# nfmoore/databricks-kubernetes-mlops-poc

Measured on NVIDIA H100. Metric: rows/sec at batch=65536x23f, higher is better.
Workload: dtype u16 ranks + f64acc

## Files before the change

databricks_kubernetes_mlops_poc_b200/csrc/b2f_api.cu:

```cuda
#include <cuda_runtime.h>
#include <dlfcn.h>
#include <limits.h>
#include <nccl.h>
#include <stdarg.h>
#include <stddef.h>
#include <stdio.h>
#include <stdlib.h>
#include <string.h>

#include <algorithm>
#include <cmath>
#include <string>
#include <thread>
#include <new>
#include <vector>

#include "../../include/b2f.h"
#include "feature_moments.cuh"
#include "forest_blob.h"
#include "forest_predict.cuh"
#include "forest_predict_tile.cuh"
#include "forest_predict_rank.cuh"
#include "forest_rank.h"
#include "tree_shap.cuh"
// ... 204 lines not shown
                const uint32_t t = N[(s * 32 + l) * 2], m = N[(s * 32 + l) * 2 + 1];
                const uint32_t feat = m >> B2F_META_FEAT_SHIFT, first = m & B2F_META_SLOT_MASK;
                const bool leaf = (first == s);
                if ((m & 0x03000000u) || feat > B2F_SENTINEL_WORD)
                    return set_err(B2F_EINVAL, "forest blob: group %u slot %u lane %u: bad meta word 0x%08x", g, s, l, m);
                if (leaf) {
                    if (!(m & B2F_META_CAT) || feat != B2F_SENTINEL_WORD || t >= gr.n_leaf_slots)
                        return set_err(B2F_EINVAL, "forest blob: group %u slot %u lane %u: malformed leaf", g, s, l);
                } else {
                    if (first <= s || first + 1 >= gr.n_slots) return set_err(B2F_EINVAL, "forest blob: group %u slot %u lane %u: child %u out of range", g, s, l, first);
                    if ((m & B2F_META_CAT) && feat >= h.n_cat && feat != B2F_SENTINEL_WORD)
                        return set_err(B2F_EINVAL, "forest blob: group %u slot %u lane %u: categorical test on numeric word", g, s, l);
                }
            }
    }
    if (expect_off != h.chunks_bytes) return set_err(B2F_EINVAL, "forest blob: chunks_bytes mismatch");
    *hdr_out = h;
    return B2F_OK;
}

extern "C" int b2f_blob_validate(const void *forest_blob, size_t nbytes) {
    b2f_blob_header h;
    return validate_blob(static_cast<const uint8_t *>(forest_blob), nbytes, &h);
}

extern "C" b2f_ranker *b2f_ranker_create(const void *forest_blob, size_t nbytes) {
    b2f_blob_header h;
    if (validate_blob(static_cast<const uint8_t *>(forest_blob), nbytes, &h) != B2F_OK) return nullptr;
    b2f_ranker *r = new (std::nothrow) b2f_ranker();
    if (!r) {
        set_err(B2F_ENOMEM, "out of host memory");
        return nullptr;
    }
    ranker_build(r, static_cast<const uint8_t *>(forest_blob), h);
    return r;
}
extern "C" void b2f_ranker_destroy(b2f_ranker *r) { delete r; }

static void fill_rank_info(const b2f_ranker *r, bool ok, b2f_rank_info *out) {
    memset(out, 0, sizeof(*out));
    out->ok = ok ? 1 : 0;
    out->row_bytes = r->row_bytes;
    out->cat_bytes = r->cat_bytes;
    out->n_cat = r->n_cat;
    out->n_num = r->n_num;
    out->depth = r->depth;
    out->n_trees = r->n_trees;
    out->layout_bytes = (int32_t)r->layout.size();
    for (int j = 0; j < 16; ++j) {
        out->cat_shift[j] = r->cat_shift[j];
        out->cat_bits[j] = r->cat_bits[j];
    }
    for (size_t k = 0; k < r->thr.size() && k < 24; ++k) out->n_thresholds[k] = (int32_t)r->thr[k].size();
    out->n_pairs = (int32_t)r->pairs.size();
    for (size_t i = 0; i < r->pairs.size() && i < 128; ++i) out->pairs[i] = r->pairs[i];
    snprintf(out->why, sizeof(out->why), "%s", r->why);
}
extern "C" int b2f_ranker_info(const b2f_ranker *r, b2f_rank_info *out) {
    if (!r || !out) return set_err(B2F_EINVAL, "null argument");
    fill_rank_info(r, r->ok, out);
    return B2F_OK;
}
extern "C" const float *b2f_ranker_thresholds(const b2f_ranker *r, int k, int32_t *count) {
    if (!r || k < 0 || k >= (int)r->thr.size()) {
        if (count) *count = 0;
        return nullptr;
    }
    if (count) *count = (int32_t)r->thr[k].size();
    return r->thr[k].data();
}
extern "C" const void *b2f_ranker_layout(const b2f_ranker *r, int64_t *nbytes) {
    if (!r || !r->ok) {
        if (nbytes) *nbytes = 0;
        return nullptr;
    }
    if (nbytes) *nbytes = (int64_t)r->layout.size();
    return r->layout.data();
}
extern "C" int b2f_ranker_rank_rows(const b2f_ranker *r, const void *rows, int64_t n, int row_format, void *ranked_out, int threads) {
    if (!r || n < 0 || (n > 0 && (!rows || !ranked_out))) return set_err(B2F_EINVAL, "bad argument");
    if (!r->ok) return set_err(B2F_EINVAL, "no rank layout for this forest (%s)", r->why);
    if (row_format != B2F_ROWS_WORDS24 && row_format != B2F_ROWS_PACKED64) return set_err(B2F_EINVAL, "rows must be B2F_ROWS_WORDS24 or B2F_ROWS_PACKED64");
    if (row_format == B2F_ROWS_PACKED64 && !(r->n_cat == 9 && r->n_num <= 14)) return set_err(B2F_EINVAL, "schema does not fit the packed 64-byte row");
    threads = (int)std::min<int64_t>(std::max(threads, 1), std::max<int64_t>(1, n / 4096));
    const uint8_t *in = static_cast<const uint8_t *>(rows);
    uint8_t *out = static_cast<uint8_t *>(ranked_out);
    if (threads == 1) {
        rank_rows_range(r, in, 0, n, row_format, out);
        return B2F_OK;
    }
    std::vector<std::thread> pool;
    for (int t = 1; t < threads; ++t) pool.emplace_back([=] { rank_rows_range(r, in, n * t / threads, n * (t + 1) / threads, row_format, out); });
    rank_rows_range(r, in, 0, n / threads, row_format, out);
    for (auto &th : pool) th.join();
    return B2F_OK;
}

template <typename OutT>
using RankKernel = void (*)(RParams, const uint8_t *, long long, OutT *, int32_t *, int);

template <int R, typename OutT>
static auto warp_kernel_r(bool smem, bool pk) {
    if (smem) return pk ? k_forest_predict<R, true, true, OutT> : k_forest_predict<R, true, false, OutT>;
    return pk ? k_forest_predict<R, false, true, OutT> : k_forest_predict<R, false, false, OutT>;
}
template <typename OutT>
static auto warp_kernel(int rows_per_warp, bool smem, bool pk) {
    if (rows_per_warp == 4) return warp_kernel_r<4, OutT>(smem, pk);
    return rows_per_warp == 2 ? warp_kernel_r<2, OutT>(smem, pk) : warp_kernel_r<1, OutT>(smem, pk);
}
template <typename OutT>
static auto tile_kernel(bool pk) {
    return pk ? k_forest_predict_tile<true, OutT> : k_forest_predict_tile<false, OutT>;
}
template <typename OutT>
static auto split_kernel(bool pk) {
    return pk ? k_forest_predict_split<2, true, OutT> : k_forest_predict_split<2, false, OutT>;
}
template <typename OutT, int D = 1>
static RankKernel<OutT> rank_kernel(const b2f_model *m) {
    if constexpr (D > 8) {
        return nullptr;
    } else {
        if (m->rp.depth != D) return rank_kernel<OutT, D + 1>(m);
        if (m->rank_stream) return k_forest_predict_rank<D, 4, true, OutT>;
        return m->rank_u == 8 ? k_forest_predict_rank<D, 8, false, OutT> : k_forest_predict_rank<D, 4, false, OutT>;
    }
}
template <typename K>
static cudaError_t set_smem_limit(K kernel, int bytes) {
    return kernel ? cudaFuncSetAttribute(kernel, cudaFuncAttributeMaxDynamicSharedMemorySize, bytes) : cudaErrorInvalidValue;
}

enum { KN_AUTO, KN_WARP, KN_TILE, KN_SPLIT };
struct EnvHooks {
    int kernel = KN_AUTO;
    bool walk_global = false;
    bool walk_smem = false;
    int64_t chunk_rows = B2F_CHUNK_ROWS;
    std::vector<int64_t> chunk_plan{768};
    int64_t split_max_rows = 2048;
    int rows_per_warp = 2;
    int64_t tile_min_rows = -1;
    int tile_warps = 0;
    bool rank_off = false;
    int rank_max_tiles = INT_MAX;
    int rank_stream = -1;
    int rank_u = 4;
    bool rank_wait_first = false;
    bool no_pdl = false;
};

static EnvHooks read_env_hooks(void) {
    EnvHooks h;
    if (const char *v = getenv("B2F_KERNEL"))
        h.kernel = !strcmp(v, "warp") ? KN_WARP : !strcmp(v, "tile") ? KN_TILE : !strcmp(v, "split") ? KN_SPLIT : KN_AUTO;
    if (const char *v = getenv("B2F_FORCE_WALK")) {
        h.walk_global = !strcmp(v, "global");
        h.walk_smem = !strcmp(v, "smem");
    }
    if (const char *v = getenv("B2F_CHUNK_ROWS"))
        if (atoll(v) >= 1024) h.chunk_rows = atoll(v);
    if (const char *v = getenv("B2F_CHUNK_PLAN")) {
        h.chunk_plan.clear();
        for (const char *q = v; *q;) {
            h.chunk_plan.push_back(atoll(q));
            while (*q && *q != ',') ++q;
            if (*q == ',') ++q;
        }
    }
    if (const char *v = getenv("B2F_SPLIT_MAX_ROWS")) h.split_max_rows = atoll(v);
    if (const char *v = getenv("B2F_ROWS_PER_WARP")) {
        const int r = atoi(v);
        if (r == 1 || r == 2 || r == 4) h.rows_per_warp = r;
    }
    if (const char *v = getenv("B2F_TILE_MIN_ROWS"))
        if (atoll(v) >= 0) h.tile_min_rows = atoll(v);
    if (const char *v = getenv("B2F_TILE_WARPS")) h.tile_warps = std::min(B2F_TILE_WARPS_MAX, std::max(1, atoi(v)));
    if (const char *v = getenv("B2F_RANK")) h.rank_off = !strcmp(v, "0");
    if (const char *v = getenv("B2F_RANK_MAX_TILES")) h.rank_max_tiles = std::max(1, atoi(v));
    if (const char *v = getenv("B2F_RANK_STREAM")) h.rank_stream = atoi(v) != 0;
    if (const char *v = getenv("B2F_RANK_U")) h.rank_u = atoi(v) == 8 ? 8 : 4;
    if (const char *v = getenv("B2F_RANK_WAIT_FIRST")) h.rank_wait_first = atoi(v) != 0;
    h.no_pdl = getenv("B2F_NO_PDL") != nullptr;
    return h;
}


struct TileTree {
    std::vector<uint32_t> nodes;
    std::vector<double> leaves;
    uint32_t depth = 0;
};

static bool extract_tree(const uint8_t *blob, const b2f_blob_header &h, const b2f_blob_group &gr, uint32_t lane, TileTree &out) {
    const uint32_t *N = reinterpret_cast<const uint32_t *>(blob + h.chunks_off + gr.chunk_off);
    const double *LV = reinterpret_cast<const double *>(blob + h.chunks_off + gr.chunk_off + (size_t)gr.n_slots * 256);
    std::vector<uint32_t> depth_of(gr.n_slots, 0);
    uint32_t reach = 0, max_leaf = 0, max_depth = 0;
    for (uint32_t s = 0; s <= reach; ++s) {
        const uint32_t t = N[(s * 32 + lane) * 2], m = N[(s * 32 + lane) * 2 + 1];
        const uint32_t feat = m >> B2F_META_FEAT_SHIFT, first = m & B2F_META_SLOT_MASK;
        const bool cat = (m & B2F_META_CAT) != 0;
        if (first >= B2F_TILE_MAX_TREE_NODES) return false;
        out.nodes.push_back(t);
        out.nodes.push_back((first << B2F_TILE_CHILD_SHIFT) | (cat ? B2F_TILE_META_CAT : 0u) | (feat << B2F_TILE_FEAT_SHIFT));
        if (first == s) {
            max_leaf = std::max(max_leaf, t);
            max_depth = std::max(max_depth, depth_of[s]);
        } else {
            reach = std::max(reach, first + 1);
            depth_of[first] = depth_of[first + 1] = depth_of[s] + 1;
        }
    }
    out.leaves.resize(max_leaf + 1);
    for (uint32_t i = 0; i <= max_leaf; ++i) out.leaves[i] = LV[i * 32 + lane];
    out.depth = max_depth;
    return true;
}

static bool build_tile_layout(const uint8_t *blob, const b2f_blob_header &h, uint32_t avail_smem, std::vector<uint8_t> &layout,
                              std::vector<TPiece> &pieces, uint32_t *slot_bytes, int *n_slots) {
    const b2f_blob_group *gt = reinterpret_cast<const b2f_blob_group *>(blob + h.groups_off);
    std::vector<TileTree> trees(h.n_trees);
    for (uint32_t t = 0; t < h.n_trees; ++t)
        if (!extract_tree(blob, h, gt[t / 32], t % 32, trees[t])) return false;
    struct UG {
        uint32_t first, count, bytes;
    };
    std::vector<UG> ugs;
    uint64_t total = 0;
    for (uint32_t t = 0; t < h.n_trees; t += B2F_TILE_U) {
        UG u{t, std::min<uint32_t>(B2F_TILE_U, h.n_trees - t), (uint32_t)sizeof(TUGroup)};
        for (uint32_t k = 0; k < B2F_TILE_U; ++k)
            u.bytes += k < u.count ? (uint32_t)(trees[t + k].nodes.size() * 4 + trees[t + k].leaves.size() * 8) : 16u;
        ugs.push_back(u);
        total += u.bytes;
    }
    uint32_t max_ug = 0;
    for (const UG &u : ugs) max_ug = std::max(max_ug, u.bytes);
    const bool fits = total + (uint64_t)(max_ug + 128) * B2F_TILE_MAX_SLOTS <= avail_smem;
    uint32_t target = fits ? (uint32_t)((total + B2F_TILE_MAX_SLOTS - 1) / B2F_TILE_MAX_SLOTS) + max_ug : 32u * 1024u;
    layout.clear();
    pieces.clear();
    size_t i = 0;
    uint32_t max_piece = 0;
    while (i < ugs.size()) {
        size_t j = i;
        uint32_t bytes = 0;
        while (j < ugs.size() && (j == i || bytes + ugs[j].bytes <= target)) bytes += ugs[j++].bytes;
        const uint32_t n_ug = (uint32_t)(j - i);
        const size_t start = layout.size();
        std::vector<uint8_t> buf((size_t)n_ug * sizeof(TUGroup));
        for (uint32_t g = 0; g < n_ug; ++g) {
            TUGroup d;
            memset(&d, 0, sizeof(d));
            for (uint32_t k = 0; k < B2F_TILE_U; ++k) {
                while (buf.size() % 8) buf.push_back(0);
                d.node_off[k] = (uint32_t)buf.size();
                if (k < ugs[i + g].count) {
                    const TileTree &tr = trees[ugs[i + g].first + k];
                    const uint8_t *np = reinterpret_cast<const uint8_t *>(tr.nodes.data());
                    buf.insert(buf.end(), np, np + tr.nodes.size() * 4);
                    d.leaf_off[k] = (uint32_t)buf.size();
                    const uint8_t *lp = reinterpret_cast<const uint8_t *>(tr.leaves.data());
                    buf.insert(buf.end(), lp, lp + tr.leaves.size() * 8);
                    d.depth = std::max(d.depth, tr.depth);
                } else {
                    const uint32_t stub[2] = {0u, (0u << B2F_TILE_CHILD_SHIFT) | B2F_TILE_META_CAT | (B2F_SENTINEL_WORD << B2F_TILE_FEAT_SHIFT)};
                    const uint8_t *sp = reinterpret_cast<const uint8_t *>(stub);
                    buf.insert(buf.end(), sp, sp + 8);
                    d.leaf_off[k] = (uint32_t)buf.size();
                    const double z = 0.0;
                    const uint8_t *zp = reinterpret_cast<const uint8_t *>(&z);
                    buf.insert(buf.end(), zp, zp + 8);
                }
            }
            memcpy(buf.data() + (size_t)g * sizeof(TUGroup), &d, sizeof(d));
        }
        while (buf.size() % 128) buf.push_back(0);
        layout.insert(layout.end(), buf.begin(), buf.end());
        pieces.push_back(TPiece{(uint32_t)start, (uint32_t)buf.size(), n_ug, 0u});
        max_piece = std::max<uint32_t>(max_piece, (uint32_t)buf.size());
        i = j;
    }
    *slot_bytes = max_piece;
    if ((size_t)max_piece * pieces.size() <= avail_smem && pieces.size() <= B2F_TILE_MAX_SLOTS) {
        *n_slots = (int)pieces.size();
    } else {
        int s = (int)std::min<uint64_t>(B2F_TILE_MAX_SLOTS, avail_smem / max_piece);
        if (s < 2) return false;
        *n_slots = s;
    }
    return true;
}

static int rank_init(b2f_model *m, const uint8_t *blob, const EnvHooks &env) {
    m->rank_ok = false;
    ranker_build(&m->rk, blob, m->hdr);
    if (!m->rk.ok) return B2F_OK;
    if (env.rank_off) return B2F_OK;
    const int64_t layout_bytes = (int64_t)m->rk.layout.size();
    const int64_t base = B2F_RANK_XS_BYTES  + (int64_t)B2F_RANK_PARTIALS * 32 * 8 + 256;
    int max_tiles = (int)std::min<int64_t>(B2F_RANK_MAX_TILES, ((int64_t)m->max_smem_optin - base - layout_bytes) / B2F_RANK_XS_BYTES);
    max_tiles = std::min(max_tiles, env.rank_max_tiles);
    m->rank_stream = env.rank_stream < 0 ? max_tiles < 8 : env.rank_stream != 0;
    int64_t forest_smem = layout_bytes;
    m->rank_u = env.rank_u;
    if (m->rank_stream) {
        m->rank_u = 4;
        const int64_t piece = 8 * (int64_t)m->rk.tree_stride;
        forest_smem = 2 * piece;
        max_tiles = (int)std::min<int64_t>(B2F_RANK_MAX_TILES, ((int64_t)m->max_smem_optin - base - forest_smem) / B2F_RANK_XS_BYTES);
        if (max_tiles < 4 || piece % 16) return B2F_OK;
    }
    CUDA_TRY(cudaMalloc(&m->d_rank_layout, (size_t)layout_bytes));
    CUDA_TRY(cudaMemcpy(m->d_rank_layout, m->rk.layout.data(), (size_t)layout_bytes, cudaMemcpyHostToDevice));
    RParams &rp = m->rp;
    memset(&rp, 0, sizeof(rp));
    rp.layout = static_cast<const uint8_t *>(m->d_rank_layout);
    rp.layout_bytes = (uint32_t)layout_bytes;
    rp.tree_stride = m->rk.tree_stride;
    rp.n_trees_padded = m->rk.n_trees_padded;
    rp.depth = m->rk.depth;
    rp.agg_mode = (int)m->hdr.agg_mode;
    rp.n_cat = m->rk.n_cat;
    rp.n_num = m->rk.n_num;
    rp.row_bytes = m->rk.row_bytes;
    rp.cat_bytes = m->rk.cat_bytes;
    rp.max_tiles = max_tiles;
    rp.groups_per_piece = 2;
    rp.piece_bytes = 8u * m->rk.tree_stride;
    rp.n_pieces = m->rk.n_trees_padded / 8;
    rp.init_raw = m->hdr.init_raw;
    rp.denom = m->hdr.denom;
    rp.threshold = m->hdr.threshold;
    rp.mul_two = 2u;
    rp.mul_64k = 65536u;
    rp.add_64k = 65535u;
    rp.n_pairs = (int)m->rk.pairs.size();
    rp.wait_first = env.rank_wait_first;
    m->rank_pdl = !env.no_pdl;
    for (int j = 0; j < 16; ++j) {
        rp.cat_shift[j] = (uint8_t)m->rk.cat_shift[j];
        rp.cat_bits[j] = (uint8_t)m->rk.cat_bits[j];
        rp.cat_start[j] = 0;
        rp.cat_mask[j] = 0ull;
    }
    for (int i = rp.n_pairs - 1; i >= 0; --i) {
        const uint32_t j = m->rk.pairs[i] >> 16, c = m->rk.pairs[i] & 0xFFFFu;
        rp.cat_start[j] = (uint8_t)i;
        rp.cat_mask[j] |= 1ull << c;
    }
    m->rank_smem_bytes = (int)(B2F_RANK_XS_BYTES + (int64_t)max_tiles * B2F_RANK_XS_BYTES + (int64_t)B2F_RANK_PARTIALS * 32 * 8 + forest_smem);
    CUDA_TRY(set_smem_limit(rank_kernel<float>(m), m->rank_smem_bytes));
    CUDA_TRY(set_smem_limit(rank_kernel<double>(m), m->rank_smem_bytes));
    m->rank_ok = true;
    return B2F_OK;
}

static int warp_init(b2f_model *m, const uint8_t *blob, const EnvHooks &env) {
    KParams &kp = m->kp;
    memset(&kp, 0, sizeof(kp));
    kp.chunks = static_cast<const uint8_t *>(m->d_blob) + m->hdr.chunks_off;
    kp.n_groups = (int)m->hdr.n_groups;
    kp.agg_mode = (int)m->hdr.agg_mode;
    kp.n_cat = (int)m->hdr.n_cat;
    kp.n_num = (int)m->hdr.n_num;
    kp.init_raw = m->hdr.init_raw;
    kp.denom = m->hdr.denom;
    kp.threshold = m->hdr.threshold;
    memcpy(kp.impute, m->hdr.impute, sizeof(kp.impute));
    const b2f_blob_group *gt = reinterpret_cast<const b2f_blob_group *>(blob + m->hdr.groups_off);
    for (uint32_t g = 0; g < m->hdr.n_groups; ++g) {
        kp.g[g].chunk_off = gt[g].chunk_off;
        kp.g[g].chunk_bytes = gt[g].chunk_bytes;
        kp.g[g].n_slots = gt[g].n_slots;
        kp.g[g].n_leaf_slots = gt[g].n_leaf_slots;
        kp.g[g].depth = gt[g].depth;
    }

    m->packed_ok = m->hdr.n_cat == 9 && m->hdr.n_num <= 14;
    for (uint32_t f = 0; f < m->hdr.n_cat; ++f)
        if (m->hdr.vocab[f] > 126) m->packed_ok = false;

    const int64_t need = (int64_t)m->hdr.chunks_bytes;
    const bool fits = need + 1024 <= (int64_t)m->max_smem_optin && !env.walk_global;
    if (env.walk_smem && !fits) return set_err(B2F_EINVAL, "B2F_FORCE_WALK=smem but forest needs %lld bytes", (long long)need);
    m->walk_mode = fits ? B2F_WALK_SMEM : B2F_WALK_GLOBAL;
    m->smem_bytes = fits ? (int)need : 0;
    if (fits)
        for (bool pk : {false, true})
            for (int r : {1, 2, 4}) {
                CUDA_TRY(set_smem_limit(warp_kernel<float>(r, true, pk), m->smem_bytes));
                CUDA_TRY(set_smem_limit(warp_kernel<double>(r, true, pk), m->smem_bytes));
            }
    m->chunk_rows = env.chunk_rows;
    m->chunk_plan = env.chunk_plan;
    m->split_max_rows = env.split_max_rows;
    if (env.kernel == KN_WARP || env.kernel == KN_TILE) m->split_max_rows = 0;
    if (env.kernel == KN_SPLIT) m->split_max_rows = INT64_MAX;
    m->rows_per_warp_max = env.rows_per_warp;
    return B2F_OK;
}

static int tile_init(b2f_model *m, const uint8_t *blob, const EnvHooks &env) {
    std::vector<uint8_t> layout;
    std::vector<TPiece> pieces;
    uint32_t slot_bytes = 0;
    int n_slots = 0;
    bool ok = false;
    int cwarps = B2F_TILE_WARPS_MIN;
    const int w_hi = env.tile_warps ? env.tile_warps : B2F_TILE_WARPS_MAX, w_lo = env.tile_warps ? env.tile_warps : B2F_TILE_WARPS_MIN;
    for (int w = w_hi; env.kernel != KN_WARP && w >= w_lo && !ok; w -= 4) {
        const uint32_t avail = (uint32_t)m->max_smem_optin - 1024u - 4096u - (uint32_t)w * B2F_TILE_XS_BYTES;
        const bool built = build_tile_layout(blob, m->hdr, avail, layout, pieces, &slot_bytes, &n_slots);
        const bool res = built && (int)pieces.size() <= n_slots;
        if (built && (res || w == w_lo)) {
            ok = true;
            cwarps = w;
        }
    }
    if (!ok) {
        if (env.kernel == KN_TILE) return set_err(B2F_EINVAL, "B2F_KERNEL=tile but the forest's trees do not fit the tile kernel's shared-memory ring");
        return B2F_OK;
    }
    CUDA_TRY(cudaMalloc(&m->d_tile_layout, layout.size()));
    CUDA_TRY(cudaMemcpy(m->d_tile_layout, layout.data(), layout.size(), cudaMemcpyHostToDevice));
    CUDA_TRY(cudaMalloc((void **)&m->d_tile_pieces, pieces.size() * sizeof(TPiece)));
    CUDA_TRY(cudaMemcpy(m->d_tile_pieces, pieces.data(), pieces.size() * sizeof(TPiece), cudaMemcpyHostToDevice));
    const KParams &kp = m->kp;
    TParams &tp = m->tp;
    memset(&tp, 0, sizeof(tp));
    tp.layout = static_cast<const uint8_t *>(m->d_tile_layout);
    tp.pieces = m->d_tile_pieces;
    tp.n_pieces = (int)pieces.size();
    tp.n_slots = n_slots;
    tp.slot_bytes = slot_bytes;
    tp.agg_mode = kp.agg_mode;
    tp.n_cat = kp.n_cat;
    tp.n_num = kp.n_num;
    tp.init_raw = kp.init_raw;
    tp.denom = kp.denom;
    tp.threshold = kp.threshold;
    memcpy(tp.impute, kp.impute, sizeof(tp.impute));
    m->tile_cwarps = cwarps;
    m->tile_smem_bytes = 4096 + cwarps * B2F_TILE_XS_BYTES + n_slots * (int)slot_bytes;
    m->tile_layout_bytes = (int64_t)layout.size();
    for (bool pk : {false, true}) {
        CUDA_TRY(set_smem_limit(tile_kernel<float>(pk), m->tile_smem_bytes));
        CUDA_TRY(set_smem_limit(tile_kernel<double>(pk), m->tile_smem_bytes));
    }
    m->tile_ok = true;
    m->tile_min_rows = (tp.n_pieces <= tp.n_slots) ? 65536 : 24576;
    if (env.tile_min_rows >= 0) m->tile_min_rows = env.tile_min_rows;
    if (env.kernel == KN_TILE) m->tile_min_rows = 1;
    return B2F_OK;
}

static int streams_init(b2f_model *m) {
    for (int s = 0; s < B2F_STREAMS; ++s) CUDA_TRY(cudaStreamCreateWithFlags(&m->slots[s].stream, cudaStreamNonBlocking));
    CUDA_TRY(cudaStreamCreateWithFlags(&m->compute, cudaStreamNonBlocking));
    CUDA_TRY(cudaFuncSetAttribute(k_feature_moments, cudaFuncAttributeMaxDynamicSharedMemorySize, B2F_MOM_SMEM));
    m->mom_blocks = m->sm_count * 3;
    CUDA_TRY(cudaMalloc(&m->d_mom_partials, (size_t)m->mom_blocks * B2F_MOM_VALUES * sizeof(double)));
    CUDA_TRY(cudaMalloc(&m->d_mom_ticket, sizeof(unsigned int)));
    CUDA_TRY(cudaMemset(m->d_mom_ticket, 0, sizeof(unsigned int)));
    CUDA_TRY(cudaMalloc(&m->d_mom_out, B2F_MOM_VALUES * sizeof(double)));
    return B2F_OK;
}

static int model_init_cuda(b2f_model *m, const uint8_t *blob, size_t nbytes) {
    const EnvHooks env = read_env_hooks();
    CUDA_TRY(cudaSetDevice(m->device));
    cudaDeviceProp prop;
    CUDA_TRY(cudaGetDeviceProperties(&prop, m->device));
    if (prop.major != 9 || prop.minor != 0)
        return set_err(B2F_ENODEV, "device %d is sm_%d%d; this library is built for sm_90a (H100) only", m->device, prop.major, prop.minor);
    m->sm_count = prop.multiProcessorCount;
    CUDA_TRY(cudaDeviceGetAttribute(&m->max_smem_optin, cudaDevAttrMaxSharedMemoryPerBlockOptin, m->device));
    CUDA_TRY(cudaMalloc(&m->d_blob, nbytes));
    CUDA_TRY(cudaMemcpy(m->d_blob, blob, nbytes, cudaMemcpyHostToDevice));
    m->forest_bytes = (int64_t)m->hdr.chunks_bytes;
    int rc = warp_init(m, blob, env);
    if (rc == B2F_OK) rc = tile_init(m, blob, env);
    if (rc == B2F_OK) rc = rank_init(m, blob, env);
    if (rc == B2F_OK) rc = streams_init(m);
    return rc;
}

extern "C" b2f_model *b2f_model_create(const void *forest_blob, size_t nbytes, int device) {
    int ndev = b2f_device_count();
    if (ndev < 0) return nullptr;
    if (device < 0 || device >= ndev) {
        set_err(B2F_EINVAL, "device %d out of range (have %d)", device, ndev);
        return nullptr;
    }
    b2f_model *m = new (std::nothrow) b2f_model();
    if (!m) {
        set_err(B2F_ENOMEM, "out of host memory");
        return nullptr;
    }
    m->device = device;
    if (validate_blob(static_cast<const uint8_t *>(forest_blob), nbytes, &m->hdr) != B2F_OK ||
        model_init_cuda(m, static_cast<const uint8_t *>(forest_blob), nbytes) != B2F_OK) {
        char keep[sizeof(g_err)];
        memcpy(keep, g_err, sizeof(keep));
        b2f_model_destroy(m);
        memcpy(g_err, keep, sizeof(keep));
        return nullptr;
    }
    return m;
}

static void explainer_free(Explainer *ex) {
    for (ExplainBuf *b = ex->slots; b <= &ex->compute; ++b) {
        if (b->out) cudaFree(b->out);
        if (b->scratch) cudaFree(b->scratch);
    }
    if (ex->d_table) cudaFree(ex->d_table);
    delete ex;
}

extern "C" void b2f_model_destroy(b2f_model *m) {
    if (!m) return;
    cudaSetDevice(m->device);
    cudaDeviceSynchronize();
    if (m->outlier) b2f_model_destroy(m->outlier);
    if (m->ex) explainer_free(m->ex);
    if (m->comm && g_nccl.CommDestroy) g_nccl.CommDestroy(m->comm);
    for (int s = 0; s < B2F_STREAMS; ++s) {
        Slot &sl = m->slots[s];
        if (sl.d_rows) cudaFree(sl.d_rows);
        if (sl.d_proba) cudaFree(sl.d_proba);
        if (sl.d_label) cudaFree(sl.d_label);
        if (sl.stream) cudaStreamDestroy(sl.stream);
    }
    for (auto &t : m->tickets)
        for (auto &e : t.ev)
            if (e) cudaEventDestroy(e);
    if (m->compute) cudaStreamDestroy(m->compute);
    if (m->d_blob) cudaFree(m->d_blob);
    if (m->d_tile_layout) cudaFree(m->d_tile_layout);
    if (m->d_tile_pieces) cudaFree(m->d_tile_pieces);
    if (m->d_rank_layout) cudaFree(m->d_rank_layout);
    if (m->d_mom_rows) cudaFree(m->d_mom_rows);
    if (m->d_mom_partials) cudaFree(m->d_mom_partials);
    if (m->d_mom_ticket) cudaFree(m->d_mom_ticket);
    if (m->d_mom_out) cudaFree(m->d_mom_out);
    if (m->d_gather) cudaFree(m->d_gather);
    if (m->d_flush) cudaFree(m->d_flush);
    delete m;
}

static int pick_rows_per_warp(const b2f_model *m, int64_t n) {
    int r = m->rows_per_warp_max;
    const int64_t warps = (int64_t)m->sm_count * B2F_PREDICT_WARPS;
    while (r > 1 && n / r < warps) r >>= 1;
    return r;
}

extern "C" int b2f_model_info(const b2f_model *m, b2f_info *out) {
    if (!m || !out) return set_err(B2F_EINVAL, "null argument");
    memset(out, 0, sizeof(*out));
    out->device = m->device;
    out->sm_count = m->sm_count;
    out->agg_mode = (int)m->hdr.agg_mode;
    out->walk_mode = m->walk_mode;
    out->n_trees = (int)m->hdr.n_trees;
    out->n_groups = (int)m->hdr.n_groups;
    out->max_depth = (int)m->hdr.max_depth;
    out->n_cat = (int)m->hdr.n_cat;
    out->n_num = (int)m->hdr.n_num;
    out->smem_bytes = m->smem_bytes;
    out->block_threads = B2F_PREDICT_THREADS;
    out->rows_per_warp = m->rows_per_warp_max;
    out->forest_bytes = m->forest_bytes;
    out->launches = m->launches + (m->outlier ? m->outlier->launches : 0);
    out->launches_tile = m->launches_tile + (m->outlier ? m->outlier->launches_tile : 0);
    out->tile_min_rows = m->tile_min_rows;
    out->tile_ok = m->tile_ok ? 1 : 0;
    out->tile_resident = (m->tile_ok && m->tp.n_pieces <= m->tp.n_slots) ? 1 : 0;
    out->packed_ok = m->packed_ok ? 1 : 0;
    out->tile_warps = m->tile_ok ? m->tile_cwarps : 0;
    out->launches_split = m->launches_split;
    out->split_max_rows = m->split_max_rows;
    out->outlier_trees = m->outlier ? (int)m->outlier->hdr.n_trees : 0;
    out->rank_ok = m->rank_ok ? 1 : 0;
    out->launches_rank = m->launches_rank;
    out->rank_smem_bytes = m->rank_ok ? m->rank_smem_bytes : 0;
    out->rank_row_bytes = m->rk.row_bytes;
    out->rank_stream = (m->rank_ok && m->rank_stream) ? 1 : 0;
    return B2F_OK;
}

extern "C" int b2f_model_rank_info(const b2f_model *m, b2f_rank_info *out) {
    if (!m || !out) return set_err(B2F_EINVAL, "null argument");
    fill_rank_info(&m->rk, m->rank_ok, out);
    if (m->rk.ok && !m->rank_ok) snprintf(out->why, sizeof(out->why), "the rank layout (%zu bytes) does not stay resident in shared memory", m->rk.layout.size());
    return B2F_OK;
}

extern "C" void *b2f_pinned_alloc(size_t nbytes) {
    void *p = nullptr;
    cudaError_t e = cudaHostAlloc(&p, nbytes ? nbytes : 1, cudaHostAllocPortable);
    if (e != cudaSuccess) {
        set_err(B2F_ENOMEM, "cudaHostAlloc(%zu) failed: %s", nbytes, cudaGetErrorString(e));
        return nullptr;
    }
    return p;
}
extern "C" void b2f_pinned_free(void *p) {
    if (p) cudaFreeHost(p);
}

enum KernelKind { KERN_RANK, KERN_TILE, KERN_SPLIT, KERN_WARP };
struct KernelChoice {
    KernelKind kind;
    int rows_per_warp = 0;
    bool smem = false;
};

static KernelChoice pick_kernel(const b2f_model *m, int64_t n, int fmt) {
    if (fmt == B2F_ROWS_RANKED) return {KERN_RANK};
    if (m->tile_ok && n >= m->tile_min_rows) return {KERN_TILE};
    if (n <= m->split_max_rows) return {KERN_SPLIT};
// ... 1018 lines not shown
```

databricks_kubernetes_mlops_poc_b200/csrc/forest_predict_rank.cuh:

```cuda
#pragma once
#include <cuda_runtime.h>
#include <stdint.h>

#include "forest_predict.cuh"
#include "forest_predict_tile.cuh"

#define B2F_RANK_THREADS 1024
#define B2F_RANK_WARPS 32
#define B2F_RANK_MAX_TILES 16
#define B2F_RANK_XS_BYTES 8192
#define B2F_RANK_PARTIALS (B2F_RANK_WARPS + B2F_RANK_MAX_TILES)

struct RParams {
    const uint8_t *layout;
    uint32_t layout_bytes;
    uint32_t tree_stride;
    int32_t n_trees_padded;
    int32_t depth;
    int32_t agg_mode;
    int32_t n_cat;
    int32_t n_num;
    int32_t row_bytes;
    int32_t cat_bytes;
    int32_t max_tiles;
    int32_t n_pieces;
    int32_t groups_per_piece;
    uint32_t piece_bytes;
    double init_raw;
    double denom;
    double threshold;
    uint32_t mul_two;
    uint32_t mul_64k;
    uint32_t add_64k;
    int32_t n_pairs;
    int32_t wait_first;
    uint8_t cat_shift[16];
    uint8_t cat_bits[16];
    uint8_t cat_start[16];
    unsigned long long cat_mask[16];
#ifdef B2F_RANK_PHASES
    unsigned long long *phases;
    int32_t phase_launch;
    int32_t phase_launches;
#endif
};

__device__ __forceinline__ void pdl_launch_dependents() { asm volatile("griddepcontrol.launch_dependents;" ::: "memory"); }
__device__ __forceinline__ void pdl_wait() { asm volatile("griddepcontrol.wait;" ::: "memory"); }

#ifdef B2F_RANK_PHASES
#define B2F_RANK_PHASE_SLOTS 8
enum { B2F_RANK_ENTRY = 0, B2F_RANK_FOREST_READY, B2F_RANK_ROWS_STAGED, B2F_RANK_WALK_DONE, B2F_RANK_WAIT_RELEASED, B2F_RANK_EXIT, B2F_RANK_SMID };
__device__ __forceinline__ void rank_phase(const RParams &p, int i) {
    if (threadIdx.x != 0 || p.phases == nullptr || p.phase_launch >= p.phase_launches) return;
    unsigned long long *q = p.phases + ((size_t)p.phase_launch * gridDim.x + blockIdx.x) * B2F_RANK_PHASE_SLOTS;
    unsigned long long t;
    asm volatile("mov.u64 %0, %%globaltimer;" : "=l"(t));
    q[i] = t;
    if (i == B2F_RANK_ENTRY) {
        uint32_t sm;
        asm volatile("mov.u32 %0, %%smid;" : "=r"(sm));
        q[B2F_RANK_SMID] = sm;
    }
}
#define RANK_PHASE(i) rank_phase(p, B2F_RANK_##i)
#else
#define RANK_PHASE(i) ((void)0)
#endif

__device__ __forceinline__ uint32_t lds_u16(uint32_t a) {
    uint32_t v;
    asm volatile("{ .reg .u16 h; ld.shared.u16 h, [%1]; cvt.u32.u16 %0, h; }" : "=r"(v) : "r"(a));
    return v;
}

template <int D, int U>
__device__ __forceinline__ void rank_walk_group(uint32_t t0, uint32_t tree_stride, uint32_t xs_lane, uint32_t m2, uint32_t m64k, uint32_t a64k,
                                                double &acc) {
    uint32_t at[U], k4[U], k8[U];
#pragma unroll
    for (int u = 0; u < U; ++u) {
        at[u] = t0 + u * tree_stride;
        k4[u] = 4u - at[u];
        k8[u] = 8u - at[u];
    }
#pragma unroll
    for (int d = 0; d < D; ++d) {
#pragma unroll
        for (int u = 0; u < U; ++u) {
            const uint32_t nw = lds32(at[u]);
            const uint32_t v = lds_u16(xs_lane | (nw & 0x1F82u));
            const uint32_t x = v * m64k + a64k;
            at[u] = at[u] * m2 + (x >= nw ? k8[u] : k4[u]);
        }
    }
#pragma unroll
    for (int u = 0; u < U; ++u) acc += lds_f64(at[u] + at[u] + k4[u] + 4u - (4u << D));
}

template <int D, int U, bool STREAM, typename OutT>
__global__ void __launch_bounds__(B2F_RANK_THREADS, 1)
    k_forest_predict_rank(const __grid_constant__ RParams p, const uint8_t *__restrict__ rows, long long n, OutT *__restrict__ proba,
                          int32_t *__restrict__ label, int ostride) {
    extern __shared__ __align__(128) uint8_t smem[];
    __shared__ __align__(8) uint64_t forest_bar[2];

    const int tid = threadIdx.x;
    const int lane = tid & 31;
    const int warp = tid >> 5;

    pdl_launch_dependents();
    RANK_PHASE(ENTRY);

    const uint32_t pad = (B2F_RANK_XS_BYTES - (smem_addr(smem) & (B2F_RANK_XS_BYTES - 1u))) & (B2F_RANK_XS_BYTES - 1u);
    uint8_t *xs_all = smem + pad;
    double *partial = reinterpret_cast<double *>(xs_all + (size_t)p.max_tiles * B2F_RANK_XS_BYTES);
    uint8_t *forest = reinterpret_cast<uint8_t *>(partial + B2F_RANK_PARTIALS * 32);

    if (tid == 0) {
        mbar_init(&forest_bar[0], 1);
        mbar_init(&forest_bar[1], 1);
        fence_mbar_init();
        fence_proxy_async();
        if constexpr (!STREAM) {
            mbar_arrive_expect_tx(&forest_bar[0], p.layout_bytes);
            for (uint32_t o = 0; o < p.layout_bytes; o += B2F_BULK_PIECE) {
                const uint32_t part = min(B2F_BULK_PIECE, p.layout_bytes - o);
                tma_bulk_g2s(forest + o, p.layout + o, part, &forest_bar[0]);
            }
        }
    }
    auto issue_piece = [&](uint32_t k) {
        const uint32_t slot = k & 1u, piece = k % (uint32_t)p.n_pieces;
        mbar_arrive_expect_tx(&forest_bar[slot], p.piece_bytes);
        tma_bulk_g2s(forest + slot * p.piece_bytes, p.layout + (size_t)piece * p.piece_bytes, p.piece_bytes, &forest_bar[slot]);
    };

    const uint32_t n_tiles = (uint32_t)((n + 31) >> 5);
    const uint32_t tq = n_tiles / gridDim.x, tr = n_tiles % gridDim.x;
    const uint32_t tile0 = blockIdx.x * tq + min(blockIdx.x, tr), cta_tiles = tq + (blockIdx.x < tr ? 1u : 0u);
    const uint32_t n_rounds = (cta_tiles + (uint32_t)p.max_tiles - 1u) / (uint32_t)p.max_tiles;
    const int groups = p.n_trees_padded / U;
    const uint32_t forest_addr = smem_addr(forest);
    const uint32_t xs_addr = smem_addr(xs_all);
    bool forest_ready = false;

    const bool wait_first = p.wait_first != 0;
    auto wait_previous = [&]() {
        pdl_wait();
        RANK_PHASE(WAIT_RELEASED);
    };
    if (wait_first) wait_previous();

    for (uint32_t round = 0; round < n_rounds; ++round) {
        const uint32_t rt0 = cta_tiles * round / n_rounds, rt1 = cta_tiles * (round + 1u) / n_rounds;
        const int T = (int)(rt1 - rt0);
        const long long row0 = (long long)(tile0 + rt0) * 32;
        const int n_rows = (int)min((long long)T * 32, n - row0);
        if (round > 0) __syncthreads();

        {
            const int items = T * 32 * 2;
            const int num_words = (p.n_num + 1) >> 1, hot_words = (p.n_pairs + 1) >> 1;
            for (int it = tid; it < items; it += B2F_RANK_THREADS) {
                const int part = it >= T * 32 ? 1 : 0, r = it - part * (T * 32);
                const uint32_t col = xs_addr + (uint32_t)(r >> 5) * B2F_RANK_XS_BYTES + (uint32_t)(r & 31) * 4u;
                const bool live = r < n_rows;
                const uint8_t *row = rows + (size_t)(row0 + (live ? r : 0)) * p.row_bytes;
                if (part == 0) {
                    const uint32_t *q = reinterpret_cast<const uint32_t *>(row + p.cat_bytes);
                    for (int w = 0; w < num_words; ++w) {
                        uint32_t v = live ? __ldg(q + w) : 0u;
                        if (2 * w + 1 >= p.n_num) v &= 0xFFFFu;
                        asm volatile("st.shared.u32 [%0], %1;" ::"r"(col + (uint32_t)w * 128u), "r"(v) : "memory");
                    }
                } else {
                    const uint32_t hot = col + (uint32_t)num_words * 128u;
                    for (int w = 0; w < hot_words; ++w) asm volatile("st.shared.u32 [%0], %1;" ::"r"(hot + (uint32_t)w * 128u), "r"(0u) : "memory");
                    if (live) {
                        unsigned long long cw = __ldg(reinterpret_cast<const uint32_t *>(row));
                        if (p.cat_bytes == 8) cw |= (unsigned long long)__ldg(reinterpret_cast<const uint32_t *>(row) + 1) << 32;
                        for (int j = 0; j < p.n_cat; ++j) {
                            const uint32_t code1 = (uint32_t)(cw >> p.cat_shift[j]) & ((1u << p.cat_bits[j]) - 1u);
                            const unsigned long long m = p.cat_mask[j];
                            if (code1 != 0u && code1 <= 64u && ((m >> (code1 - 1u)) & 1ull)) {
                                const uint32_t slot = (uint32_t)p.cat_start[j] + (uint32_t)__popcll(m & ((1ull << (code1 - 1u)) - 1ull));
                                asm volatile("st.shared.u16 [%0], %1;" ::"r"(hot + (slot >> 1) * 128u + (slot & 1u) * 2u), "h"((uint16_t)1) : "memory");
                            }
                        }
                    }
                }
            }
        }
        if constexpr (STREAM) {
            if (tid == 0) {
                issue_piece(round * (uint32_t)p.n_pieces);
                if (p.n_pieces > 1) issue_piece(round * (uint32_t)p.n_pieces + 1u);
            }
        }
        __syncthreads();
        RANK_PHASE(ROWS_STAGED);
        if constexpr (!STREAM) {
            if (!forest_ready) {
                mbar_wait(&forest_bar[0], 0);
                forest_ready = true;
                RANK_PHASE(FOREST_READY);
            }
        }

        if constexpr (STREAM) {
            const int GP = p.groups_per_piece;
            const bool mine = warp < T * GP;
            const uint32_t xs_lane = xs_addr + (uint32_t)(warp / GP) * B2F_RANK_XS_BYTES + (uint32_t)lane * 4u;
            const uint32_t g_off = (uint32_t)(warp % GP) * U * p.tree_stride;
            double acc = 0.0;
            for (int piece = 0; piece < p.n_pieces; ++piece) {
                const uint32_t k = round * (uint32_t)p.n_pieces + (uint32_t)piece;
                mbar_wait(&forest_bar[k & 1u], (k >> 1) & 1u);
                if (k == 0) RANK_PHASE(FOREST_READY);
                if (mine) rank_walk_group<D, U>(forest_addr + (k & 1u) * p.piece_bytes + g_off, p.tree_stride, xs_lane, p.mul_two, p.mul_64k, p.add_64k, acc);
                __syncthreads();
                if (tid == 0 && piece + 2 < p.n_pieces) issue_piece(k + 2u);
            }
            if (mine) partial[warp * 32 + lane] = acc;
            __syncthreads();
            RANK_PHASE(WALK_DONE);
            if (round == 0 && !wait_first) wait_previous();
            for (int r = tid; r < n_rows; r += B2F_RANK_THREADS) {
                const int t = r >> 5, ln = r & 31;
                double s = p.agg_mode == B2F_AGG_GBDT_LOGISTIC ? p.init_raw : 0.0;
                for (int g = 0; g < GP; ++g) s += partial[(t * GP + g) * 32 + ln];
                double p1;
                int lab;
                aggregate(p.agg_mode, p.agg_mode == B2F_AGG_GBDT_LOGISTIC ? 0.0 : p.init_raw, p.denom, p.threshold, s, p1, lab);
                const long long row = row0 + r;
                if (proba) proba[row * ostride_p(ostride)] = (OutT)p1;
                if (label) label[row * ostride_l(ostride)] = lab;
            }
            continue;
        }

        {
            const int units = T * groups;
            int u = warp * units / B2F_RANK_WARPS;
            const int u_end = (warp + 1) * units / B2F_RANK_WARPS;
            while (u < u_end) {
                const int t = u / groups;
                const int g_end = min(groups, u_end - t * groups);
                const uint32_t xs_lane = xs_addr + (uint32_t)t * B2F_RANK_XS_BYTES + (uint32_t)lane * 4u;
                double acc = 0.0;
                for (int g = u - t * groups; g < g_end; ++g)
                    rank_walk_group<D, U>(forest_addr + (uint32_t)(g * U) * p.tree_stride, p.tree_stride, xs_lane, p.mul_two, p.mul_64k, p.add_64k, acc);
                partial[(warp + t) * 32 + lane] = acc;
                u = t * groups + g_end;
            }
        }
        __syncthreads();
        RANK_PHASE(WALK_DONE);
        if (round == 0 && !wait_first) wait_previous();

        for (int r = tid; r < n_rows; r += B2F_RANK_THREADS) {
            const int t = r >> 5, ln = r & 31;
            const int units = T * groups;
            const int w_first = (int)(((uint32_t)(t * groups + 1) * B2F_RANK_WARPS + (uint32_t)units - 1u) / (uint32_t)units) - 1;
            const int w_last = (int)(((uint32_t)((t + 1) * groups) * B2F_RANK_WARPS + (uint32_t)units - 1u) / (uint32_t)units) - 1;
            double s = p.agg_mode == B2F_AGG_GBDT_LOGISTIC ? p.init_raw : 0.0;
            for (int w = w_first; w <= w_last; ++w)
                if ((w + 1) * units / B2F_RANK_WARPS > w * units / B2F_RANK_WARPS) s += partial[(w + t) * 32 + ln];
            double p1;
            int lab;
            aggregate(p.agg_mode, p.agg_mode == B2F_AGG_GBDT_LOGISTIC ? 0.0 : p.init_raw, p.denom, p.threshold, s, p1, lab);
            const long long row = row0 + r;
            if (proba) proba[row * ostride_p(ostride)] = (OutT)p1;
            if (label) label[row * ostride_l(ostride)] = lab;
        }
    }
    if constexpr (!STREAM) {
        if (!forest_ready) mbar_wait(&forest_bar[0], 0);
    }
#ifdef B2F_RANK_PHASES
    __syncthreads();
#endif
    RANK_PHASE(EXIT);
}
```

Before: 3.790 billion.

## Serve top two tree levels from kernel parameters and skip padded tree groups

Puts the root and depth-1 node words of each tree in the grid-constant parameter block (up to 288 trees), so the first two levels of the non-streaming walk read from constant memory instead of shared memory. Shared-memory sizing and the forest copy now cover only the walked groups rather than the padded layout, which may allow more row tiles. The walk loop also stops at the real group count, skipping padded trees. In exchange the parameter block grows to nearly 4 KB, and divergent per-lane selection of kids may serialize constant-cache reads.

```diff
diff --git a/databricks_kubernetes_mlops_poc_b200/csrc/b2f_api.cu b/databricks_kubernetes_mlops_poc_b200/csrc/b2f_api.cu
--- a/databricks_kubernetes_mlops_poc_b200/csrc/b2f_api.cu
+++ b/databricks_kubernetes_mlops_poc_b200/csrc/b2f_api.cu
@@ -530,11 +530,15 @@
     if (env.rank_off) return B2F_OK;
     const int64_t layout_bytes = (int64_t)m->rk.layout.size();
     const int64_t base = B2F_RANK_XS_BYTES  + (int64_t)B2F_RANK_PARTIALS * 32 * 8 + 256;
-    int max_tiles = (int)std::min<int64_t>(B2F_RANK_MAX_TILES, ((int64_t)m->max_smem_optin - base - layout_bytes) / B2F_RANK_XS_BYTES);
+    m->rank_u = env.rank_u;
+    const int n_groups = (m->rk.n_trees + m->rank_u - 1) / m->rank_u;
+    const int64_t walked_bytes = (int64_t)n_groups * m->rank_u * m->rk.tree_stride;
+    int max_tiles = (int)std::min<int64_t>(B2F_RANK_MAX_TILES, ((int64_t)m->max_smem_optin - base - walked_bytes) / B2F_RANK_XS_BYTES);
     max_tiles = std::min(max_tiles, env.rank_max_tiles);
-    m->rank_stream = env.rank_stream < 0 ? max_tiles < 8 : env.rank_stream != 0;
-    int64_t forest_smem = layout_bytes;
-    m->rank_u = env.rank_u;
+    const bool top_fits = m->rk.n_trees <= B2F_RANK_TOP_TREES;
+    if (env.rank_stream == 0 && !top_fits) return B2F_OK;
+    m->rank_stream = env.rank_stream < 0 ? (max_tiles < 8 || !top_fits) : env.rank_stream != 0;
+    int64_t forest_smem = walked_bytes;
     if (m->rank_stream) {
         m->rank_u = 4;
         const int64_t piece = 8 * (int64_t)m->rk.tree_stride;
@@ -547,9 +551,17 @@
     RParams &rp = m->rp;
     memset(&rp, 0, sizeof(rp));
     rp.layout = static_cast<const uint8_t *>(m->d_rank_layout);
-    rp.layout_bytes = (uint32_t)layout_bytes;
+    rp.layout_bytes = (uint32_t)(m->rank_stream ? layout_bytes : walked_bytes);
     rp.tree_stride = m->rk.tree_stride;
     rp.n_trees_padded = m->rk.n_trees_padded;
+    rp.n_groups = n_groups;
+    if (!m->rank_stream) {
+        for (int t = 0; t < m->rk.n_trees; ++t) {
+            const uint32_t *nodes = reinterpret_cast<const uint32_t *>(m->rk.layout.data() + (size_t)t * m->rk.tree_stride);
+            rp.top_root[t] = nodes[0];
+            if (m->rk.depth >= 2) rp.top_kids[t] = make_uint2(nodes[1], nodes[2]);
+        }
+    }
     rp.depth = m->rk.depth;
     rp.agg_mode = (int)m->hdr.agg_mode;
     rp.n_cat = m->rk.n_cat;
diff --git a/databricks_kubernetes_mlops_poc_b200/csrc/forest_predict_rank.cuh b/databricks_kubernetes_mlops_poc_b200/csrc/forest_predict_rank.cuh
--- a/databricks_kubernetes_mlops_poc_b200/csrc/forest_predict_rank.cuh
+++ b/databricks_kubernetes_mlops_poc_b200/csrc/forest_predict_rank.cuh
@@ -10,12 +10,14 @@
 #define B2F_RANK_MAX_TILES 16
 #define B2F_RANK_XS_BYTES 8192
 #define B2F_RANK_PARTIALS (B2F_RANK_WARPS + B2F_RANK_MAX_TILES)
+#define B2F_RANK_TOP_TREES 288
 
 struct RParams {
     const uint8_t *layout;
     uint32_t layout_bytes;
     uint32_t tree_stride;
     int32_t n_trees_padded;
+    int32_t n_groups;
     int32_t depth;
     int32_t agg_mode;
     int32_t n_cat;
@@ -43,7 +45,10 @@
     int32_t phase_launch;
     int32_t phase_launches;
 #endif
+    uint32_t top_root[B2F_RANK_TOP_TREES];
+    uint2 top_kids[B2F_RANK_TOP_TREES];
 };
+static_assert(sizeof(RParams) + 5 * 8 <= 4096, "rank kernel parameters exceed 4 KB");
 
 __device__ __forceinline__ void pdl_launch_dependents() { asm volatile("griddepcontrol.launch_dependents;" ::: "memory"); }
 __device__ __forceinline__ void pdl_wait() { asm volatile("griddepcontrol.wait;" ::: "memory"); }
@@ -74,13 +79,14 @@
     return v;
 }
 
-template <int D, int U>
-__device__ __forceinline__ void rank_walk_group(uint32_t t0, uint32_t tree_stride, uint32_t xs_lane, uint32_t m2, uint32_t m64k, uint32_t a64k,
-                                                double &acc) {
+template <int D, int U, bool TOP>
+__device__ __forceinline__ void rank_walk_group(const RParams &p, int tree0, uint32_t t0, uint32_t xs_lane, double &acc) {
+    const uint32_t m2 = p.mul_two, m64k = p.mul_64k, a64k = p.add_64k;
     uint32_t at[U], k4[U], k8[U];
+    bool second0[U];
 #pragma unroll
     for (int u = 0; u < U; ++u) {
-        at[u] = t0 + u * tree_stride;
+        at[u] = t0 + u * p.tree_stride;
         k4[u] = 4u - at[u];
         k8[u] = 8u - at[u];
     }
@@ -88,10 +94,20 @@
     for (int d = 0; d < D; ++d) {
 #pragma unroll
         for (int u = 0; u < U; ++u) {
-            const uint32_t nw = lds32(at[u]);
+            uint32_t nw;
+            if (TOP && d == 0) {
+                nw = p.top_root[tree0 + u];
+            } else if (TOP && d == 1) {
+                const uint2 kids = p.top_kids[tree0 + u];
+                nw = second0[u] ? kids.y : kids.x;
+            } else {
+                nw = lds32(at[u]);
+            }
             const uint32_t v = lds_u16(xs_lane | (nw & 0x1F82u));
             const uint32_t x = v * m64k + a64k;
-            at[u] = at[u] * m2 + (x >= nw ? k8[u] : k4[u]);
+            const bool second = x >= nw;
+            if (d == 0) second0[u] = second;
+            at[u] = at[u] * m2 + (second ? k8[u] : k4[u]);
         }
     }
 #pragma unroll
@@ -218,7 +234,7 @@
                 const uint32_t k = round * (uint32_t)p.n_pieces + (uint32_t)piece;
                 mbar_wait(&forest_bar[k & 1u], (k >> 1) & 1u);
                 if (k == 0) RANK_PHASE(FOREST_READY);
-                if (mine) rank_walk_group<D, U>(forest_addr + (k & 1u) * p.piece_bytes + g_off, p.tree_stride, xs_lane, p.mul_two, p.mul_64k, p.add_64k, acc);
+                if (mine) rank_walk_group<D, U, false>(p, 0, forest_addr + (k & 1u) * p.piece_bytes + g_off, xs_lane, acc);
                 __syncthreads();
                 if (tid == 0 && piece + 2 < p.n_pieces) issue_piece(k + 2u);
             }
@@ -249,8 +265,8 @@
                 const int g_end = min(groups, u_end - t * groups);
                 const uint32_t xs_lane = xs_addr + (uint32_t)t * B2F_RANK_XS_BYTES + (uint32_t)lane * 4u;
                 double acc = 0.0;
-                for (int g = u - t * groups; g < g_end; ++g)
-                    rank_walk_group<D, U>(forest_addr + (uint32_t)(g * U) * p.tree_stride, p.tree_stride, xs_lane, p.mul_two, p.mul_64k, p.add_64k, acc);
+                for (int g = u - t * groups; g < min(g_end, p.n_groups); ++g)
+                    rank_walk_group<D, U, true>(p, g * U, forest_addr + (uint32_t)(g * U) * p.tree_stride, xs_lane, acc);
                 partial[(warp + t) * 32 + lane] = acc;
                 u = t * groups + g_end;
             }
```

Measured after the change: 3.986 billion, median of 6. 1.05x the previous value.
